# anand-12/botorch

Hardware: AMD Instinct MI355X
Metric: acq-evals/sec (q x restarts x MC), qEI forward (higher is better)
Workload: dtype f64; 1 GPU; C3 qEI forward: SingleTaskGP n=4096 d=6, q=16, 512 restarts/GPU, 512 Sobol MC samples, best_f = max(Y) - 1.5; n=4096, d=6, q=16, restarts_per_gpu=512, mc=512, parallelism=restart-sharded x1

## Files before the change

### botorch_amd/csrc/post.hip

```cpp
#include "common.h"

#include <algorithm>
#include <cstdlib>
#include <map>
#include <mutex>
#include <tuple>
#include <vector>

namespace {

constexpr int PC = 128;
constexpr int PI = 128;
constexpr int PK = 16;
constexpr int PLD = 144;
constexpr int DP = 8;
constexpr int kSlots = 512;
constexpr int kTileDoubles = 32 * 64;
#ifndef KXT_K
#define KXT_K 16
#endif

template <int KIND, int ND>
__device__ __forceinline__ double eval_kernel_row(const double (&xi)[ND], const double* __restrict__ Xt,
                                                  int n, int k, double outputscale, bool ivalid) {
  if (k >= n || !ivalid) return 0.0;
  const double* xt = Xt + (int64_t)k * DP;
  double d2 = 0.0;
#pragma unroll
  for (int t = 0; t < ND; ++t) {
    const double df = xi[t] - xt[t];
    d2 = fma(df, df, d2);
  }
#ifdef BO_PROBE_CHEAP_KERNEL
  return outputscale * d2 * 0.0;
#else
  return outputscale * kernel_from_d2<KIND>(d2);
#endif
}

__host__ __device__ __forceinline__ int splitk_chunks(int ci, int n, int kc_len) {
  const int e = ci * PC + PC;
  const int kfull = n < e ? n : e;
  return (kfull + kc_len - 1) / kc_len;
}
__host__ __device__ __forceinline__ int64_t splitk_base(int ci, int n, int kc_len) {
  int64_t s = 0;
  for (int c = 0; c < ci; ++c) s += splitk_chunks(c, n, kc_len);
  return s;
}

__device__ __forceinline__ void post_store_rt(const v4d (&acc)[8], int ci, int row0, int lane,
                                              int nI, double* __restrict__ Rt) {
  const int c0 = ci * PC;
  const int nrows_pad = nI * PI;
#pragma unroll
  for (int ct = 0; ct < 8; ++ct)
#pragma unroll
    for (int r = 0; r < 4; ++r) {
      const int c = c0 + ct * 16 + mfma_row(lane, r);
      Rt[(int64_t)c * nrows_pad + row0 + mfma_col(lane)] = acc[ct][r];
    }
}

__device__ __forceinline__ void post_epilogue(const v4d (&acc)[8], int ci, int row0, int lane,
                                              int n, const double* __restrict__ beta, int nI,
                                              double* __restrict__ Spart,
                                              double* __restrict__ mpart) {
  const int c0 = ci * PC;
  const int nrows16 = nI * (PI / 16);
  const int nrows_pad = nI * PI;
  v4d P = v4d_zero();
#pragma unroll
  for (int ct = 0; ct < 8; ++ct)
#pragma unroll
    for (int r = 0; r < 4; ++r) P = mfma_f64(acc[ct][r], acc[ct][r], P);
  double* sp = Spart + ((int64_t)ci * nrows16 + row0 / 16) * 256;
#pragma unroll
  for (int r = 0; r < 4; ++r) sp[mfma_row(lane, r) * 16 + mfma_col(lane)] = P[r];

  double m = 0.0;
#pragma unroll
  for (int ct = 0; ct < 8; ++ct)
#pragma unroll
    for (int r = 0; r < 4; ++r) {
      const int c = c0 + ct * 16 + mfma_row(lane, r);
      m = fma(acc[ct][r], (c < n) ? beta[c] : 0.0, m);
    }
  m += __shfl_xor(m, 16);
  m += __shfl_xor(m, 32);
  if (lane < 16) mpart[(int64_t)ci * nrows_pad + row0 + lane] = m;
}

struct FusedDx {
  const double* dmean;
  const double* dcov;
  const double* alpha;
  const double* Xq;
  const double* Xt;
  double ystd, outputscale;
  int B, q, Qp;
  double* part;
};

constexpr int POST_MAXM = 8;
struct PostMembers {
  const double* U[POST_MAXM];
  const double* beta[POST_MAXM];
  const double* Kt[POST_MAXM];
  double* Spart[POST_MAXM];
  double* mpart[POST_MAXM];
  double* Rt[POST_MAXM];
  int nm;
};

#ifndef BO_POST_PAIRED_REV
#define BO_POST_PAIRED_REV 1
#endif
#ifndef BO_USTORE_ALWAYS
#define BO_USTORE_ALWAYS 1
#endif
template <int KIND, int ND, bool SPLIT, bool CROSS, bool PRE = false, bool LOWERK = false,
          bool FUSEDX = false>
__global__ __launch_bounds__(256, 2) void post_partials_kernel(
    const double* __restrict__ Xq, int nrows, const double* __restrict__ Xt, int n,
    const double* __restrict__ U, int64_t ldu, const double* __restrict__ beta,
    double outputscale, int nC, int nI, double* __restrict__ Spart, double* __restrict__ mpart,
    double* __restrict__ Rt, const int4* __restrict__ segs, const int* __restrict__ wg_off,
    double* __restrict__ work, const double* __restrict__ Qc, int rq, int64_t ldq,
    double* __restrict__ Cx, const double* __restrict__ Kt, int grouped, FusedDx fx = FusedDx{},
    int rt_blk = 0, PostMembers pm = PostMembers{}) {
  __shared__ __attribute__((aligned(16))) double Us[2][PK][PLD];
  __shared__ __attribute__((aligned(16))) double Ks[2][PK][PLD];

  const int bid = blockIdx.x;
  int ci = 0, ii = 0, kbeg = 0, kend = 0;
  int ci_long = 0, ci_short = 0;
  if constexpr (SPLIT) {
  } else if (grouped == 2) {
    const int xcd = bid & 7;
    const int slot = bid >> 3;
    const int t = (slot >> 6) * 8 + xcd;
    const int w = slot & 63;
    const int nIG = nI >> 3;
    const int p = t / nIG;
    if (p >= (nC >> 4)) return;
    ci_long = ((nC >> 3) - 1 - p) * 8 + 7 - (w & 7);
    ci_short = p * 8 + (w & 7);
    ii = (t % nIG) * 8 + (w >> 3);
  } else if (grouped) {
    const int xcd = bid & 7;
    const int slot = bid >> 3;
    const int t = (slot >> 6) * 8 + xcd;
    const int w = slot & 63;
    const int nIG = nI >> 3;
    const int cg = (nC >> 3) - 1 - t / nIG;
    if (cg < 0) return;
    ci = cg * 8 + 7 - (w & 7);
    ii = (t % nIG) * 8 + (w >> 3);
    kend = min(n, ci * PC + PC);
  } else {
    const int xcd = bid & 7;
    const int slot = bid >> 3;
    const int jj = slot / nI;
    ii = slot - jj * nI;
    const int pos = jj * 8 + xcd;
    if (pos >= nC) return;
    ci = nC - 1 - pos;
    kend = min(n, ci * PC + PC);
  }
  if (LOWERK && !SPLIT && grouped != 2) {
    ci = nC - 1 - ci;
    kbeg = ci * PC;
    kend = n;
  }
  const double* const U_all = U;
  const double* const beta_all = beta;
  const double* const Kt_all = Kt;
  double* const Spart_all = Spart;
  double* const mpart_all = mpart;
  double* const Rt_all = Rt;
  int sbeg = 0, send = 1;
  if constexpr (SPLIT) {
    sbeg = wg_off[bid];
    send = wg_off[bid + 1];
  } else {
    if (grouped == 2) send = 2;
  }
  for (int sidx = sbeg; sidx < send; ++sidx) {
  int chunk = -1;
  if (!SPLIT && grouped == 2) {
    ci = sidx == 0 ? ci_long : ci_short;
    kbeg = 0;
    kend = min(n, ci * PC + PC);
    if constexpr (LOWERK) {
      ci = nC - 1 - ci;
      kbeg = ci * PC;
      kend = n;
    }
  }
  int mem = 0;
  if constexpr (SPLIT) {
    const int4 sg = segs[sidx];
    ci = sg.x & 0xffff;
    ii = sg.x >> 16;
    kbeg = sg.y & 0xffffff;
    mem = sg.y >> 24;
    kend = sg.z;
    chunk = sg.w;
  }
  const bool memb = SPLIT && pm.nm > 0;
  const double* U = memb ? pm.U[mem] : U_all;
  const double* beta = memb ? pm.beta[mem] : beta_all;
  const double* Kt = memb ? pm.Kt[mem] : Kt_all;
  double* Spart = memb ? pm.Spart[mem] : Spart_all;
  double* mpart = memb ? pm.mpart[mem] : mpart_all;
  double* Rt = memb ? pm.Rt[mem] : Rt_all;
  const int c0 = ci * PC;
  const int i0 = ii * PI;
  const int nsteps = (kend - kbeg + PK - 1) / PK;
  const bool rev = BO_POST_PAIRED_REV && !SPLIT && grouped == 2 && ((sidx == 1) != LOWERK);
  const int kfirst = rev ? kbeg + (nsteps - 1) * PK : kbeg;
  const int kdir = rev ? -PK : PK;

  const int tid = threadIdx.x;
  const int lane = tid & 63;
  const int wave = tid >> 6;

  const int ti = tid & (PI - 1);
  const int kh = __builtin_amdgcn_readfirstlane(tid >> 7);
  const bool ivalid = (i0 + ti) < nrows;
  double xi[ND];
#pragma unroll
  for (int t = 0; t < ND; ++t) xi[t] = ivalid ? Xq[(int64_t)(i0 + ti) * DP + t] : 0.0;

  v4d acc[8][2];
#pragma unroll
  for (int a = 0; a < 8; ++a) {
    acc[a][0] = v4d_zero();
    acc[a][1] = v4d_zero();
  }
  const bool cross = CROSS;
  v4d accx[2] = {v4d_zero(), v4d_zero()};
  double qa[4] = {0.0, 0.0, 0.0, 0.0};
  const bool qrow = CROSS && (lane & 15) < rq;
#define BO_LOAD_Q(K0)                                                              \
  if (cross) {                                                                     \
    _Pragma("unroll") for (int ks = 0; ks < 4; ++ks) {                            \
      const int kk = (K0) + ks * 4 + (lane >> 4);                                  \
      qa[ks] = (qrow && kk < n) ? Qc[(int64_t)(lane & 15) * ldq + kk] : 0.0;       \
    }                                                                              \
  }

  double u0x, u0y, u1x, u1y, u2x, u2y, u3x, u3y;
  double kv[8];
  const int urow = tid >> 6;
  const int ucol = c0 + 2 * (tid & 63);
#define BO_LOAD_U(K0)                                                             \
  {                                                                               \
    const double* src = U + (int64_t)((K0) + urow) * ldu + ucol;                  \
    const double2 v0 = *reinterpret_cast<const double2*>(src);                    \
    const double2 v1 = *reinterpret_cast<const double2*>(src + 4 * ldu);          \
    const double2 v2 = *reinterpret_cast<const double2*>(src + 8 * ldu);          \
    const double2 v3 = *reinterpret_cast<const double2*>(src + 12 * ldu);         \
    u0x = v0.x; u0y = v0.y; u1x = v1.x; u1y = v1.y;                               \
    u2x = v2.x; u2y = v2.y; u3x = v3.x; u3y = v3.y;                               \
  }
#define BO_STORE(BUF)                                                             \
  {                                                                               \
    double* dst = &Us[BUF][urow][2 * (tid & 63)];                                 \
    *reinterpret_cast<double2*>(dst) = make_double2(u0x, u0y);                    \
    *reinterpret_cast<double2*>(dst + 4 * PLD) = make_double2(u1x, u1y);          \
    *reinterpret_cast<double2*>(dst + 8 * PLD) = make_double2(u2x, u2y);          \
    *reinterpret_cast<double2*>(dst + 12 * PLD) = make_double2(u3x, u3y);         \
    if (!PRE) {                                                                   \
      _Pragma("unroll") for (int kk = 0; kk < 8; ++kk) Ks[BUF][kh * 8 + kk][ti] = kv[kk]; \
    }                                                                             \
  }

#define BO_KVAL(K)                                                                         \
  (PRE ? Kt[(int64_t)(K) * (nI * PI) + i0 + ti]                                            \
       : eval_kernel_row<KIND, ND>(xi, Xt, n, (K), outputscale, ivalid))
  double bc[2][4], bn[2][4];
  const double* ktw = PRE ? Kt + i0 + wave * 32 + (lane & 15) + (int64_t)(lane >> 4) * (nI * PI)
                          : nullptr;
  const double* ktb = FUSEDX ? Kt + (int64_t)((i0 + wave * 32) >> 4) * 256 + lane : nullptr;
#define BO_LOAD_B(K0, DST)                                                          \
  _Pragma("unroll") for (int it = 0; it < 2; ++it)                                 \
    _Pragma("unroll") for (int ks = 0; ks < 4; ++ks)                              \
      DST[it][ks] = FUSEDX ? ktb[((int64_t)((K0) >> 4) * (nI * (PI / 16)) + it) * 256 + ks * 64] \
                           : ktw[(int64_t)((K0) + 4 * ks) * (nI * PI) + it * 16];
  BO_LOAD_U(kfirst);
  if (PRE) {
    BO_LOAD_B(kfirst, bc);
  } else {
#pragma unroll
    for (int kk = 0; kk < 8; ++kk)
      kv[kk] = BO_KVAL(kfirst + kh * 8 + kk);
  }
  BO_STORE(0);
  __syncthreads();
#define BO_KSTEP(XLOAD, XMFMA)                                                       \
  {                                                                                  \
    const int cur = t & 1;                                                           \
    const bool more = t + 1 < nsteps;                                                \
    const int knext = kfirst + (more ? t + 1 : t) * kdir;                            \
    XLOAD                                                                            \
    BO_LOAD_U(knext);                                                                \
    if (PRE) { BO_LOAD_B(knext, bn); }                                               \
    _Pragma("unroll") for (int ks = 0; ks < PK / 4; ++ks) {                         \
      const int kr = ks * 4 + (lane >> 4);                                           \
      double a[8], b[2];                                                             \
      _Pragma("unroll") for (int ct = 0; ct < 8; ++ct) a[ct] = Us[cur][kr][ct * 16 + (lane & 15)]; \
      _Pragma("unroll") for (int it = 0; it < 2; ++it)                              \
        b[it] = PRE ? bc[it][ks] : Ks[cur][kr][wave * 32 + it * 16 + (lane & 15)];   \
      _Pragma("unroll") for (int ct = 0; ct < 8; ++ct)                              \
        _Pragma("unroll") for (int it = 0; it < 2; ++it)                            \
          acc[ct][it] = FUSEDX ? mfma_f64(b[it], a[ct], acc[ct][it])                \
                               : mfma_f64(a[ct], b[it], acc[ct][it]);                \
      XMFMA                                                                          \
      if (!PRE) {                                                                    \
        kv[2 * ks] = BO_KVAL(knext + kh * 8 + 2 * ks);                              \
        kv[2 * ks + 1] = BO_KVAL(knext + kh * 8 + 2 * ks + 1);                      \
      }                                                                              \
    }                                                                                \
    if (BO_USTORE_ALWAYS || more) BO_STORE(cur ^ 1);                                 \
    if (PRE) {                                                                       \
      _Pragma("unroll") for (int it = 0; it < 2; ++it)                              \
        _Pragma("unroll") for (int ks = 0; ks < 4; ++ks) bc[it][ks] = bn[it][ks];   \
    }                                                                                \
    __syncthreads();                                                                 \
  }
  int t = 0;
  if (cross) {
    const int tc = min(nsteps, c0 / PK);
    const int t0 = rev ? 0 : tc, t1 = rev ? nsteps - tc : nsteps;
    for (; t < t0; ++t) BO_KSTEP(, )
    for (; t < t1; ++t)
      BO_KSTEP(BO_LOAD_Q(kfirst + t * kdir),
               accx[0] = mfma_f64(qa[ks], b[0], accx[0]);
               accx[1] = mfma_f64(qa[ks], b[1], accx[1]);)
    for (; t < nsteps; ++t) BO_KSTEP(, )
  } else {
    for (; t < nsteps; ++t) BO_KSTEP(, )
  }
#undef BO_KSTEP
#undef BO_KVAL
#undef BO_LOAD_U
#undef BO_STORE
#undef BO_LOAD_Q
#undef BO_LOAD_B
  if (cross) {
    const int nrows_pad = nI * PI;
#pragma unroll
    for (int it = 0; it < 2; ++it)
#pragma unroll
      for (int r = 0; r < 4; ++r) {
        const int j = mfma_row(lane, r);
        if (j < rq)
          Cx[((int64_t)ci * rq + j) * nrows_pad + i0 + wave * 32 + it * 16 + mfma_col(lane)] =
              accx[it][r];
      }
  }

  if constexpr (FUSEDX) {
    const int ncol = lane & 15, grp = lane >> 4;
    const double s2 = fx.ystd * fx.ystd;
    const int nrows_pad = nI * PI;
    double* xc_s = &Us[0][0][0];
    double* al_s = xc_s + PC * DP;
    double* xa_s = al_s + PC;
    for (int e = tid; e < PC * DP; e += 256) {
      const int c = c0 + e / DP;
      xc_s[e] = c < n ? fx.Xt[(int64_t)c * DP + (e % DP)] : 0.0;
      xa_s[e] = fx.Xq[(int64_t)i0 * DP + e];
    }
    if (tid < PC) al_s[tid] = (c0 + tid) < n ? fx.alpha[c0 + tid] : 0.0;
    __syncthreads();
#pragma unroll
    for (int it = 0; it < 2; ++it) {
      const int row16 = i0 + wave * 32 + it * 16;
      const int rl = wave * 32 + it * 16;
      double ga[4];
#pragma unroll
      for (int r = 0; r < 4; ++r) {
        const int ra = row16 + ncol, rj = row16 + grp + 4 * r;
        const int ba = ra / fx.Qp, bj = rj / fx.Qp;
        const int aa = ra - ba * fx.Qp, jj = rj - bj * fx.Qp;
        ga[r] = (ba == bj && ba < fx.B && aa < fx.q && jj < fx.q)
                    ? s2 * (fx.dcov[((int64_t)ba * fx.q + aa) * fx.q + jj] +
                            fx.dcov[((int64_t)ba * fx.q + jj) * fx.q + aa])
                    : 0.0;
      }
      double dmu[4];
#pragma unroll
      for (int r = 0; r < 4; ++r) {
        const int ra = row16 + grp + 4 * r;
        const int b = ra / fx.Qp, aa = ra - b * fx.Qp;
        dmu[r] = (b < fx.B && aa < fx.q) ? fx.ystd * fx.dmean[(int64_t)b * fx.q + aa] : 0.0;
      }
#pragma unroll
      for (int h = 0; h < 2; ++h) {
        double dx[2][ND];
#pragma unroll
        for (int rr = 0; rr < 2; ++rr)
#pragma unroll
          for (int t = 0; t < ND; ++t) dx[rr][t] = 0.0;
#pragma unroll
        for (int ct = 0; ct < 8; ++ct) {
          v4d gw = v4d_zero();
#pragma unroll
          for (int r = 0; r < 4; ++r) gw = mfma_f64(ga[r], acc[ct][it][r], gw);
          const int cl = ct * 16 + ncol;
          const double al = al_s[cl];
          const bool cv = c0 + cl < n;
#pragma unroll
          for (int rr = 0; rr < 2; ++rr) {
            const int r = 2 * h + rr;
            const double D = cv ? fma(dmu[r], al, -gw[r]) : 0.0;
            const double* xa = xa_s + (rl + grp + 4 * r) * DP;
            const double* xc = xc_s + cl * DP;
            double diff[ND];
            double d2 = 0.0;
#pragma unroll
            for (int t = 0; t < ND; ++t) {
              diff[t] = xa[t] - xc[t];
              d2 = fma(diff[t], diff[t], d2);
            }
            const double f = D * dkernel_factor<KIND>(d2, fx.outputscale);
#pragma unroll
            for (int t = 0; t < ND; ++t) dx[rr][t] = fma(f, diff[t], dx[rr][t]);
          }
        }
#pragma unroll
        for (int rr = 0; rr < 2; ++rr)
#pragma unroll
          for (int t = 0; t < ND; ++t) {
            double v = dx[rr][t];
            v += __shfl_xor(v, 1);
            v += __shfl_xor(v, 2);
            v += __shfl_xor(v, 4);
            v += __shfl_xor(v, 8);
            dx[rr][t] = v;
          }
        if (ncol == 0) {
#pragma unroll
          for (int rr = 0; rr < 2; ++rr) {
            double* o = fx.part + ((int64_t)ci * nrows_pad + row16 + grp + 4 * (2 * h + rr)) * DP;
#pragma unroll
            for (int t = 0; t < ND; ++t) o[t] = dx[rr][t];
          }
        }
      }
    }
    __syncthreads();
  } else if (SPLIT && chunk >= 0) {
#pragma unroll
    for (int it = 0; it < 2; ++it) {
      double* w = work + ((int64_t)chunk * (PI / 16) + wave * 2 + it) * kTileDoubles + lane;
#pragma unroll
      for (int ct = 0; ct < 8; ++ct)
#pragma unroll
        for (int r = 0; r < 4; ++r) w[(ct * 4 + r) * 64] = acc[ct][it][r];
    }
  } else {
    const int nrows16 = nI * (PI / 16);
    const int nrows_pad = nI * PI;
    if (Rt != nullptr && rt_blk) {
#pragma unroll
      for (int ct = 0; ct < 8; ++ct)
#pragma unroll
        for (int it = 0; it < 2; ++it) {
          double* blk = Rt + ((int64_t)((c0 >> 4) + ct) * nrows16 +
                              ((i0 + wave * 32 + it * 16) >> 4)) * 256 + lane;
#pragma unroll
          for (int r = 0; r < 4; ++r) blk[r * 64] = acc[ct][it][r];
        }
    } else if (Rt != nullptr) {
#pragma unroll
      for (int ct = 0; ct < 8; ++ct)
#pragma unroll
        for (int it = 0; it < 2; ++it)
#pragma unroll
          for (int r = 0; r < 4; ++r) {
            const int c = c0 + ct * 16 + mfma_row(lane, r);
            const int i = i0 + wave * 32 + it * 16 + mfma_col(lane);
            Rt[(int64_t)c * nrows_pad + i] = acc[ct][it][r];
          }
    }
    if constexpr (!LOWERK) {
#pragma unroll
    for (int it = 0; it < 2; ++it) {
      v4d P = v4d_zero();
#pragma unroll
      for (int ct = 0; ct < 8; ++ct)
#pragma unroll
        for (int r = 0; r < 4; ++r) P = mfma_f64(acc[ct][it][r], acc[ct][it][r], P);
      const int row0 = i0 + wave * 32 + it * 16;
      double* sp = Spart + ((int64_t)ci * nrows16 + row0 / 16) * 256;
#pragma unroll
      for (int r = 0; r < 4; ++r) sp[mfma_row(lane, r) * 16 + mfma_col(lane)] = P[r];
      double m = 0.0;
#pragma unroll
      for (int ct = 0; ct < 8; ++ct)
#pragma unroll
        for (int r = 0; r < 4; ++r) {
          const int c = c0 + ct * 16 + mfma_row(lane, r);
          m = fma(acc[ct][it][r], (c < n) ? beta[c] : 0.0, m);
        }
      m += __shfl_xor(m, 16);
      m += __shfl_xor(m, 32);
      if (lane < 16) mpart[(int64_t)ci * nrows_pad + row0 + lane] = m;
    }
    }
  }
  }
}

struct RowsFromX {
  const double* X;
  const double* ls;
  int B, q, d, Qp;
  double* Xq_out;
};

struct KxtMembers {
  const double* ls[8];
  const double* Xt[8];
  double os[8];
  double* Xq[8];
  double* Kt[8];
  int nm;
};

template <int KIND, int ND, int KK = KXT_K, bool FROMX = false>
__global__ __launch_bounds__(256) void kxt_build_kernel(const double* __restrict__ Xq, int nrows,
                                                        const double* __restrict__ Xt, int n,
                                                        int np, int nrows_pad, double outputscale,
                                                        double* __restrict__ Kt,
                                                        RowsFromX rx = RowsFromX{},
                                                        KxtMembers km = KxtMembers{}) {
  if (km.nm > 0) {
    const int m = blockIdx.z;
    rx.ls = km.ls[m];
    rx.Xq_out = km.Xq[m];
    Xt = km.Xt[m];
    outputscale = km.os[m];
    Kt = km.Kt[m];
  }
  const int i = blockIdx.x * 256 + threadIdx.x;
  const int k0 = blockIdx.y * KK;
  const bool iv = i < nrows;
  double xi[ND];
  if constexpr (FROMX) {
    const int b = i / rx.Qp, a = i - (i / rx.Qp) * rx.Qp;
    const bool real = iv && b < rx.B && a < rx.q;
#pragma unroll
    for (int t = 0; t < ND; ++t)
      xi[t] = (real && t < rx.d) ? rx.X[((int64_t)b * rx.q + a) * rx.d + t] / rx.ls[t] : 0.0;
    if (blockIdx.y == 0 && i < nrows_pad) {
#pragma unroll
      for (int t = 0; t < DP; ++t)
        rx.Xq_out[(int64_t)i * DP + t] =
            (real && t < rx.d) ? rx.X[((int64_t)b * rx.q + a) * rx.d + t] / rx.ls[t] : 0.0;
    }
  } else {
#pragma unroll
    for (int t = 0; t < ND; ++t) xi[t] = iv ? Xq[(int64_t)i * DP + t] : 0.0;
  }
  if (i >= nrows_pad) return;
#pragma unroll 4
  for (int kk = 0; kk < KK; ++kk) {
    const int k = k0 + kk;
    if (k < np) Kt[(int64_t)k * nrows_pad + i] = eval_kernel_row<KIND, ND>(xi, Xt, n, k, outputscale, iv);
  }
}

__global__ __launch_bounds__(256) void post_splitk_reduce_kernel(
    const double* __restrict__ work, const int4* __restrict__ red, int n, int nI,
    const double* __restrict__ beta_all, double* __restrict__ Spart_all,
    double* __restrict__ mpart_all, double* __restrict__ Rt_all, PostMembers pm = PostMembers{}) {
  __shared__ double part[3][32][64];
  const int4 r4 = red[blockIdx.x / (PI / 16)];
  const int sub = blockIdx.x % (PI / 16);
  const int ci = r4.x & 0xffffff, rt = r4.y * (PI / 16) + sub;
  const int mem = r4.x >> 24;
  const bool memb = pm.nm > 0;
  const double* beta = memb ? pm.beta[mem] : beta_all;
  double* Spart = memb ? pm.Spart[mem] : Spart_all;
  double* mpart = memb ? pm.mpart[mem] : mpart_all;
  double* Rt = memb ? pm.Rt[mem] : Rt_all;
  const int lane = threadIdx.x & 63;
  const int wave = threadIdx.x >> 6;
  v4d acc[8];
#pragma unroll
  for (int ct = 0; ct < 8; ++ct) acc[ct] = v4d_zero();
  const int cend = r4.z + r4.w;
  int c = r4.z + wave;
  for (; c + 4 < cend; c += 8) {
    const double* w0 = work + ((int64_t)c * (PI / 16) + sub) * kTileDoubles + lane;
    const double* w1 = w0 + 4 * (PI / 16) * kTileDoubles;
    double v0[32], v1[32];
#pragma unroll
    for (int e = 0; e < 32; ++e) {
      v0[e] = w0[e * 64];
      v1[e] = w1[e * 64];
    }
#pragma unroll
    for (int ct = 0; ct < 8; ++ct)
#pragma unroll
      for (int r = 0; r < 4; ++r) acc[ct][r] += v0[ct * 4 + r];
#pragma unroll
    for (int ct = 0; ct < 8; ++ct)
#pragma unroll
      for (int r = 0; r < 4; ++r) acc[ct][r] += v1[ct * 4 + r];
  }
  if (c < cend) {
    const double* w = work + ((int64_t)c * (PI / 16) + sub) * kTileDoubles + lane;
#pragma unroll
    for (int ct = 0; ct < 8; ++ct)
#pragma unroll
      for (int r = 0; r < 4; ++r) acc[ct][r] += w[(ct * 4 + r) * 64];
  }
  if (wave > 0) {
#pragma unroll
    for (int ct = 0; ct < 8; ++ct)
#pragma unroll
      for (int r = 0; r < 4; ++r) part[wave - 1][ct * 4 + r][lane] = acc[ct][r];
  }
  __syncthreads();
  if (wave != 0) return;
#pragma unroll
  for (int w = 0; w < 3; ++w)
#pragma unroll
    for (int ct = 0; ct < 8; ++ct)
#pragma unroll
      for (int r = 0; r < 4; ++r) acc[ct][r] += part[w][ct * 4 + r][lane];
  if (Rt != nullptr) post_store_rt(acc, ci, rt * 16, lane, nI, Rt);
  if (Spart != nullptr) post_epilogue(acc, ci, rt * 16, lane, n, beta, nI, Spart, mpart);
}

template <int KIND>
__global__ __launch_bounds__(256) void post_dx_reduce_kernel(
    const double* __restrict__ part, int nC, int nrows_pad, int q, int Qp, int d,
    const double* __restrict__ Xq, const double* __restrict__ dcov,
    const double* __restrict__ ls, double outputscale, double ystd, double* __restrict__ dX) {
  const int b = blockIdx.x;
  const int tid = threadIdx.x;
  if (tid >= q * d) return;
// ... 1156 lines not shown
```

Before: 1.871 billion acq-evals/s.

## Use triple-buffered U ring with one mid-step barrier and skip zero diagonal MFMAs

For the precomputed-K path, the U tile staging moves from a double buffer to a three-slot LDS ring. The next tile is stored and synchronised halfway through each k-step, with a prefetched first fragment, so each step needs only one barrier and global loads overlap more of the MFMA work. Address arithmetic is strength-reduced into running pointers. On diagonal k-steps the MFMAs for column tiles that fall entirely in the zero triangle of the triangular factor are skipped, using a wave-uniform bound. This costs more LDS (a third U buffer), which may lower occupancy, and adds branch logic whose triangle bounds must be exactly right.

```diff
diff --git a/botorch_amd/csrc/post.hip b/botorch_amd/csrc/post.hip
--- a/botorch_amd/csrc/post.hip
+++ b/botorch_amd/csrc/post.hip
@@ -118,6 +118,9 @@
 #endif
 #ifndef BO_USTORE_ALWAYS
 #define BO_USTORE_ALWAYS 1
+#endif
+#ifndef BO_POST_RING
+#define BO_POST_RING 1
 #endif
 template <int KIND, int ND, bool SPLIT, bool CROSS, bool PRE = false, bool LOWERK = false,
           bool FUSEDX = false>
@@ -129,7 +132,8 @@
     double* __restrict__ work, const double* __restrict__ Qc, int rq, int64_t ldq,
     double* __restrict__ Cx, const double* __restrict__ Kt, int grouped, FusedDx fx = FusedDx{},
     int rt_blk = 0, PostMembers pm = PostMembers{}) {
-  __shared__ __attribute__((aligned(16))) double Us[2][PK][PLD];
+  constexpr bool RING = PRE && BO_POST_RING;
+  __shared__ __attribute__((aligned(16))) double Us[RING ? 3 : 2][PK][PLD];
   __shared__ __attribute__((aligned(16))) double Ks[2][PK][PLD];
 
   const int bid = blockIdx.x;
@@ -289,61 +293,124 @@
     _Pragma("unroll") for (int ks = 0; ks < 4; ++ks)                              \
       DST[it][ks] = FUSEDX ? ktb[((int64_t)((K0) >> 4) * (nI * (PI / 16)) + it) * 256 + ks * 64] \
                            : ktw[(int64_t)((K0) + 4 * ks) * (nI * PI) + it * 16];
-  BO_LOAD_U(kfirst);
-  if (PRE) {
-    BO_LOAD_B(kfirst, bc);
+  const int64_t ustep = (int64_t)kdir * ldu, bstep = (int64_t)kdir * (nI * PI);
+  const double* up = U + (int64_t)(kfirst + urow) * ldu + ucol;
+  const double* bp = FUSEDX ? ktb + (int64_t)(kfirst >> 4) * (nI * (PI / 16)) * 256
+                            : (PRE ? ktw + (int64_t)kfirst * (nI * PI) : nullptr);
+#define BO_LOAD_UP()                                                              \
+  {                                                                               \
+    const double2 v0 = *reinterpret_cast<const double2*>(up);                     \
+    const double2 v1 = *reinterpret_cast<const double2*>(up + 4 * ldu);           \
+    const double2 v2 = *reinterpret_cast<const double2*>(up + 8 * ldu);           \
+    const double2 v3 = *reinterpret_cast<const double2*>(up + 12 * ldu);          \
+    u0x = v0.x; u0y = v0.y; u1x = v1.x; u1y = v1.y;                               \
+    u2x = v2.x; u2y = v2.y; u3x = v3.x; u3y = v3.y;                               \
+  }
+#define BO_LOAD_BP(DST)                                                            \
+  _Pragma("unroll") for (int it = 0; it < 2; ++it)                                 \
+    _Pragma("unroll") for (int ks = 0; ks < 4; ++ks)                              \
+      DST[it][ks] = FUSEDX ? bp[it * 256 + ks * 64]                                \
+                           : bp[(int64_t)(4 * ks) * (nI * PI) + it * 16];
+  double an[8];
+  int stage = 0;
+  if (RING) {
+    BO_LOAD_UP();
+    BO_LOAD_BP(bc);
+    BO_STORE(0);
+    if (nsteps > 1) { up += ustep; bp += bstep; }
+    BO_LOAD_UP();
+    __syncthreads();
+#pragma unroll
+    for (int ct = 0; ct < 8; ++ct) an[ct] = Us[0][lane >> 4][ct * 16 + (lane & 15)];
   } else {
-#pragma unroll
-    for (int kk = 0; kk < 8; ++kk)
-      kv[kk] = BO_KVAL(kfirst + kh * 8 + kk);
-  }
-  BO_STORE(0);
-  __syncthreads();
-#define BO_KSTEP(XLOAD, XMFMA)                                                       \
+    BO_LOAD_U(kfirst);
+    if (PRE) {
+      BO_LOAD_B(kfirst, bc);
+    } else {
+#pragma unroll
+      for (int kk = 0; kk < 8; ++kk)
+        kv[kk] = BO_KVAL(kfirst + kh * 8 + kk);
+    }
+    BO_STORE(0);
+    __syncthreads();
+  }
+#define BO_KSTEP(XLOAD, XMFMA, DIAG)                                                 \
   {                                                                                  \
-    const int cur = t & 1;                                                           \
+    const int cur = RING ? stage : (t & 1);                                          \
+    const int nxt = RING ? (stage == 2 ? 0 : stage + 1) : (cur ^ 1);                 \
     const bool more = t + 1 < nsteps;                                                \
     const int knext = kfirst + (more ? t + 1 : t) * kdir;                            \
+    const int kd = kfirst + t * kdir - c0;                                           \
+    const int ctb = (DIAG) ? __builtin_amdgcn_readfirstlane(                         \
+                                 LOWERK ? (kd + PK - 1) >> 4 : max(kd, 0) >> 4)      \
+                           : 0;                                                      \
     XLOAD                                                                            \
-    BO_LOAD_U(knext);                                                                \
-    if (PRE) { BO_LOAD_B(knext, bn); }                                               \
+    if (RING) {                                                                      \
+      BO_LOAD_BP(bn);                    \
+    } else {                                                                         \
+      BO_LOAD_U(knext);                                                              \
+      if (PRE) { BO_LOAD_B(knext, bn); }                                             \
+    }                                                                                \
     _Pragma("unroll") for (int ks = 0; ks < PK / 4; ++ks) {                         \
+      if (RING && ks == PK / 8) {                                                    \
+        BO_STORE(nxt);       \
+        __syncthreads();                                                             \
+        if (t + 2 < nsteps) { up += ustep; bp += bstep; }                            \
+        BO_LOAD_UP();                   \
+      }                                                                              \
       const int kr = ks * 4 + (lane >> 4);                                           \
       double a[8], b[2];                                                             \
-      _Pragma("unroll") for (int ct = 0; ct < 8; ++ct) a[ct] = Us[cur][kr][ct * 16 + (lane & 15)]; \
+      _Pragma("unroll") for (int ct = 0; ct < 8; ++ct)                              \
+        a[ct] = (RING && ks == 0) ? an[ct] : Us[cur][kr][ct * 16 + (lane & 15)];     \
       _Pragma("unroll") for (int it = 0; it < 2; ++it)                              \
         b[it] = PRE ? bc[it][ks] : Ks[cur][kr][wave * 32 + it * 16 + (lane & 15)];   \
       _Pragma("unroll") for (int ct = 0; ct < 8; ++ct)                              \
-        _Pragma("unroll") for (int it = 0; it < 2; ++it)                            \
-          acc[ct][it] = FUSEDX ? mfma_f64(b[it], a[ct], acc[ct][it])                \
-                               : mfma_f64(a[ct], b[it], acc[ct][it]);                \
+        if (!(DIAG) || (LOWERK ? ct <= ctb : ct >= ctb)) {                           \
+          _Pragma("unroll") for (int it = 0; it < 2; ++it)                          \
+            acc[ct][it] = FUSEDX ? mfma_f64(b[it], a[ct], acc[ct][it])              \
+                                 : mfma_f64(a[ct], b[it], acc[ct][it]);              \
+        }                                                                            \
       XMFMA                                                                          \
       if (!PRE) {                                                                    \
         kv[2 * ks] = BO_KVAL(knext + kh * 8 + 2 * ks);                              \
         kv[2 * ks + 1] = BO_KVAL(knext + kh * 8 + 2 * ks + 1);                      \
       }                                                                              \
     }                                                                                \
-    if (BO_USTORE_ALWAYS || more) BO_STORE(cur ^ 1);                                 \
+    if (RING) {                                                                      \
+      _Pragma("unroll") for (int ct = 0; ct < 8; ++ct)                              \
+        an[ct] = Us[nxt][lane >> 4][ct * 16 + (lane & 15)];                          \
+      stage = nxt;                                                                   \
+    } else if (BO_USTORE_ALWAYS || more) {                                           \
+      BO_STORE(cur ^ 1);                                                             \
+    }                                                                                \
     if (PRE) {                                                                       \
       _Pragma("unroll") for (int it = 0; it < 2; ++it)                              \
         _Pragma("unroll") for (int ks = 0; ks < 4; ++ks) bc[it][ks] = bn[it][ks];   \
     }                                                                                \
-    __syncthreads();                                                                 \
+    if (!RING) __syncthreads();                                                      \
   }
   int t = 0;
   if (cross) {
     const int tc = min(nsteps, c0 / PK);
     const int t0 = rev ? 0 : tc, t1 = rev ? nsteps - tc : nsteps;
-    for (; t < t0; ++t) BO_KSTEP(, )
+    for (; t < t0; ++t) BO_KSTEP(, , 0)
     for (; t < t1; ++t)
       BO_KSTEP(BO_LOAD_Q(kfirst + t * kdir),
                accx[0] = mfma_f64(qa[ks], b[0], accx[0]);
-               accx[1] = mfma_f64(qa[ks], b[1], accx[1]);)
-    for (; t < nsteps; ++t) BO_KSTEP(, )
+               accx[1] = mfma_f64(qa[ks], b[1], accx[1]);, 1)
+    for (; t < nsteps; ++t) BO_KSTEP(, , 0)
   } else {
-    for (; t < nsteps; ++t) BO_KSTEP(, )
-  }
+    const int a0 = LOWERK ? 0 : min(nsteps, max(0, (c0 + PK - kbeg + PK - 1) / PK));
+    const int a1 = LOWERK ? min(nsteps, max(0, (c0 + PC - 2 * PK + 1 - kbeg + PK - 1) / PK)) : nsteps;
+    const int d0 = rev ? nsteps - a1 : a0, d1 = rev ? nsteps - a0 : a1;
+    for (; t < d0; ++t) BO_KSTEP(, , 0)
+    for (; t < d1; ++t) BO_KSTEP(, , 1)
+    for (; t < nsteps; ++t) BO_KSTEP(, , 0)
+  }
+  if (RING) __syncthreads();
 #undef BO_KSTEP
+#undef BO_LOAD_UP
+#undef BO_LOAD_BP
 #undef BO_KVAL
 #undef BO_LOAD_U
 #undef BO_STORE
```

Measured after the change: 1.982 billion acq-evals/s (median of 6 runs). 1.06x the previous value.
